# IsaacTroche1/MPC_ARPO_Project

Measured on AMD Instinct MI355X. Metric: MPC-QP solves/sec @ N=20, 6-state CW, batch=65536; ADMM iters to 1e-4, higher is better.
Workload: dtype f64

## Files before the change

mpc_arpo_project_amd/csrc/engine.hip:

```cpp
#include <hip/hip_runtime.h>

#include <algorithm>
#include <cmath>
#include <cstdio>
#include <cstdlib>
#include <cstring>
#include <string>
#include <vector>

#include "../../include/mpcqp.h"
#include "dev_plan.hpp"
#include "host_abi.hpp"
#include "symbolic.hpp"

using namespace mpcqp;

#pragma clang fp contract(off)

#define OSQP_INFTY 1e30
#define RHO_MIN 1e-06
#define RHO_MAX 1e06
#define RHO_EQ_OVER_RHO_INEQ 1e03
#define RHO_TOL 1e-04
#define MIN_SCALING 1e-04
// ... 1452 lines not shown
#pragma unroll
  for (int r = 0; r < RN; ++r) {
    const int j = lane + 64 * r;
    const double di = 1. / D[r];
    if (j < n) {
      v[P.S_DT + j] = di;
      qw[j] = (S.q[r] * cinv) * di;
    }
  }
  LDS_FENCE();
  unscale_p_r(v, P.S_P, P.nnzP, ra, ca, cinv, lane, Pw);
}

template <class Cx, int RN, int RM>
__device__ __forceinline__ void scale_bounds(const KParams& p, int inst, bool rebound, Inst<RN, RM>& S,
                                             const Slab& sb, const Cx& C, const double (&D)[RN],
                                             const double (&E)[RM]) {
  const DevPlan& P = p.pl;
  const int n = P.n, m = P.m, lane = C.lane;
  S.cinv = 1. / S.c;
  const double thr = OSQP_INFTY * MIN_SCALING;
  const double* Eold = p.Ecls + (size_t)inst * m;
  S.ct = 0;
#pragma unroll
  for (int r = 0; r < RM; ++r) {
    const int i = lane + 64 * (r + C.zo);
    const double ec = (rebound && i < m) ? Eold[i] : E[r];
    const double lc = S.l[r] * ec, uc = S.u[r] * ec;
    const uint32_t t = (lc < -thr && uc > thr) ? CT_FREE : ((uc - lc < RHO_TOL) ? CT_EQ : CT_INEQ);
    S.ct |= t << (2 * r);
    const double eci = 1. / ec;
    const double lb = rebound ? lc * eci : S.l[r], ub = rebound ? uc * eci : S.u[r];
    S.l[r] = lb * E[r];
    S.u[r] = ub * E[r];
    S.Einv[r] = 1. / E[r];
    if (i < m) sb.E[i] = E[r];
  }
#pragma unroll
  for (int r = 0; r < RN; ++r) {
    const int j = lane + 64 * (r + C.xo);
    S.Dinv[r] = 1. / D[r];
    if (j < n) sb.D[j] = D[r];
  }
}
template <int RN, int RM>
__device__ __forceinline__ void scale_finish(const KParams& p, int inst, bool rebound, Inst<RN, RM>& S,
                                             const Slab& sb, double* v, double* mvw, int lane,
                                             const double (&D)[RN], const double (&E)[RM]) {
  const DevPlan& P = p.pl;
  scale_bounds(p, inst, rebound, S, sb, One{lane, mvw}, D, E);
  LDS_FENCE();
  {
    const int cnt = P.nnzP + P.nnzA;
    constexpr int U = 8;
    for (int k0 = 0; k0 < cnt; k0 += 64 * U) {
      double x[U];
#pragma unroll
      for (int u = 0; u < U; ++u) {
        const int k = k0 + 64 * u + lane;
        x[u] = v[P.S_P + (k < cnt ? k : 0)];
      }
#pragma unroll
      for (int u = 0; u < U; ++u) {
        const int k = k0 + 64 * u + lane;
        if (k < cnt) mvw[P.MV + k] = x[u];
      }
    }
    if (lane == 0) mvw[P.MVZ] = 0.0;
  }
  LDS_FENCE();
  if (P.mv_slab) __builtin_amdgcn_fence(__ATOMIC_SEQ_CST, "workgroup");
}

#ifdef MPCQP_TIMING
#define TTAIL_PARAM , unsigned long long* tacc, unsigned long long t_tl
#define TTAIL_ARG(t) , tacc, t
#else
#define TTAIL_PARAM
#define TTAIL_ARG(t)
#endif
template <class Cx, int RN, int RM>
__device__ __forceinline__ void store_solution(const KParams& p, int inst, const Inst<RN, RM>& S,
                                               const Slab& sb, double* v, Cx& C, int status, int iter,
                                               int rho_updates TTAIL_PARAM) {
  const DevPlan& P = p.pl;
  const int n = P.n, m = P.m, lane = C.lane;
  const bool sol = has_solution(status);
  double obj = 0.0;
  if (sol) {
    double* xb = v + P.W;
    const double* mv = C.mv(v);
    LDS_FENCE();
#pragma unroll
    for (int r = 0; r < RN; ++r)
      if (lane + 64 * (r + C.xo) < n) xb[lane + 64 * (r + C.xo)] = S.x[r];
    C.sync(p, v);
    double part = 0.0;
    for (int k = C.tid(); k < P.nnzP; k += Cx::THREADS) {
      const int i = P.Pi[k], j = P.Pcol[k];
      const double pk = mv[P.MV + k];
      part += (i == j) ? .5 * pk * xb[i] * xb[i] : pk * xb[i] * xb[j];
    }
#pragma unroll
    for (int r = 0; r < RN; ++r)
      if (lane + 64 * (r + C.xo) < n) part += S.q[r] * S.x[r];
    obj = xch_sum(p, v, C, wave_sum(part)) * S.cinv;
  } else if (status == MPCQP_PRIMAL_INFEASIBLE || status == MPCQP_PRIMAL_INFEASIBLE_INACCURATE) {
    obj = OSQP_INFTY;
  } else if (status == MPCQP_DUAL_INFEASIBLE || status == MPCQP_DUAL_INFEASIBLE_INACCURATE) {
    obj = -OSQP_INFTY;
  }
  const double qnan = __builtin_nan("");
#pragma unroll
  for (int r = 0; r < RN; ++r) {
    const int j = lane + 64 * (r + C.xo);
    if (j < n) {
      if (p.x_out) p.x_out[(size_t)inst * n + j] = sol ? sb.D[j] * S.x[r] : qnan;
      p.xs[(size_t)inst * n + j] = sol ? S.x[r] : 0.0;
    }
  }
#pragma unroll
  for (int r = 0; r < RM; ++r) {
    const int i = lane + 64 * (r + C.zo);
    if (i < m) {
      const double Ei = sb.E[i];
      if (p.y_out) p.y_out[(size_t)inst * m + i] = sol ? (Ei * S.y[r]) * S.cinv : qnan;
      p.zs[(size_t)inst * m + i] = sol ? S.z[r] : 0.0;
      p.ys[(size_t)inst * m + i] = sol ? S.y[r] : 0.0;
      p.Ecls[(size_t)inst * m + i] = Ei;
    }
  }
  T_END(T_TAIL, t_tl);
#ifdef MPCQP_TIMING
  if (C.first() && p.timing)
    for (int k = 0; k < T_NSLOT; ++k) atomicAdd(p.timing + k, tacc[k]);
#endif
  if (C.first()) {
    p.rho_state[inst] = S.rho;
    p.has_state[inst] = 1;
    if (p.info.status) p.info.status[inst] = status;
    if (p.info.iter) p.info.iter[inst] = iter;
    if (p.info.rho_updates) p.info.rho_updates[inst] = rho_updates;
    if (p.info.obj_val) p.info.obj_val[inst] = obj;
    if (p.info.pri_res) p.info.pri_res[inst] = S.pri_res;
    if (p.info.dua_res) p.info.dua_res[inst] = S.dua_res;
    if (p.info.rho) p.info.rho[inst] = S.rho;
  }
}

#ifndef MPCQP_OPAQUE_LANE_RN
#define MPCQP_OPAQUE_LANE_RN 2
#endif
enum { KM_LDS = 0, KM_MATPF = 1, KM_MVG = 2, KM_MREG = 3 };
template <int RN, int RM, bool PAIRED, int KM, int RP>
__device__ __forceinline__ void solve_instance(const KParams& p, int inst, double* v, double* scr,
                                               int lane) {
  constexpr bool MATPF = KM == KM_MATPF, MVG = KM == KM_MVG, MREG = KM == KM_MREG;
  constexpr bool CARRY = RP == RP_CARRY;
  static_assert(!CARRY || KM == KM_LDS, "the carried record pipeline is the KM_LDS kernel's");
  const DevPlan& P = p.pl;
  const int n = P.n, m = P.m;
  const Slab sb = slab_of(P, scr);
  double* const mv = MVG ? sb.MV : v;
  One W{lane, mv};
  Inst<RN, RM> S;
  const int hs = p.has_state[inst];
  const Drift dr = drift_of(p, inst);
#ifdef MPCQP_TIMING
  unsigned long long tacc[T_NSLOT] = {};
#endif
  T_BEGIN(t_sc);
  {
    double D[RN], E[RM];
    scale_problem<RN, RM>(p, inst, dr, S, v, lane, D, E TACC_ARG);
    T_BEGIN(t_sf);
    scale_finish<RN, RM>(p, inst, dr.rebound, S, sb, v, mv, lane, D, E);
    if (lane == 0) {
      p.dsel[inst] = dr.sel;
      p.pend[inst] = 0;
    }
    T_END(T_SCFIN, t_sf);
  }
  T_END(T_SCALE, t_sc);
  S.rho = (hs != 0) ? p.rho_state[inst] : p.rho0;
  set_rho(S);
  T_BEGIN(t_f0);
  MatRegs M;
  assemble_and_factor<RN, RM>(p, sb, v, mv, lane, S);
  if constexpr (MREG) {
    LDS_FENCE();
    load_mats(P.fwdm, P.nfwd, (uint32_t)lane, v, M.m[0]);
    load_mats(P.bwdm, P.nbwd, (uint32_t)lane, v, M.m[1]);
  }
  T_END(T_FACTOR, t_f0);
  T_COUNT(T_NFACT);

  const bool warm = p.s.warm_start && hs != 0;
  if (warm && hs == 1) {
#pragma unroll
    for (int r = 0; r < RN; ++r) {
      const int j = lane + 64 * r;
      S.x[r] = j < n ? p.xs[(size_t)inst * n + j] : 0.0;
    }
#pragma unroll
    for (int r = 0; r < RM; ++r) {
      const int i = lane + 64 * r;
      S.z[r] = i < m ? p.zs[(size_t)inst * m + i] : 0.0;
      S.y[r] = i < m ? p.ys[(size_t)inst * m + i] : 0.0;
    }
  } else if (warm && hs == 2) {
#pragma unroll
    for (int r = 0; r < RN; ++r) {
      const int j = lane + 64 * r;
      S.x[r] = j < n ? S.Dinv[r] * p.xs[(size_t)inst * n + j] : 0.0;
    }
#pragma unroll
    for (int r = 0; r < RM; ++r) {
      const int i = lane + 64 * r;
      S.y[r] = i < m ? (S.Einv[r] * p.ys[(size_t)inst * m + i]) * S.c : 0.0;
    }
    double* xb = v + P.W;
    LDS_FENCE();
#pragma unroll
    for (int r = 0; r < RN; ++r)
      if (lane + 64 * r < n) xb[lane + 64 * r] = S.x[r];
    LDS_FENCE();
    double az[RM];
    ell_mv<RM, ELL_KA>(P.eA, mv, xb, az, W, W.zo, W.stage(P, v));
#pragma unroll
    for (int r = 0; r < RM; ++r) S.z[r] = lane + 64 * r < m ? az[r] : 0.0;
    LDS_FENCE();
  } else {
#pragma unroll
    for (int r = 0; r < RN; ++r) S.x[r] = 0.0;
#pragma unroll
    for (int r = 0; r < RM; ++r) S.z[r] = 0.0, S.y[r] = 0.0;
  }
  S.pri_res = S.dua_res = 0.0;

  int wsx[RN], wsz[RM];
#pragma unroll
  for (int r = 0; r < RN; ++r) wsx[r] = (int)P.wsx[lane + 64 * r];
#pragma unroll
  for (int r = 0; r < RM; ++r) wsz[r] = (int)P.wsz[lane + 64 * r];
  constexpr int coff = 64 * (RN + RM);
  const uint32_t wcp = P.wcopy[lane], bcp = P.bcopy[lane];
  constexpr bool MASK_REGS = RN < 4;
  constexpr int NMK = MASK_REGS ? RN + RM : 1;
  uint32_t wmk[NMK], bmk[NMK];
#pragma unroll
  for (int r = 0; r < NMK; ++r) {
    wmk[r] = 0u - ((wcp >> r) & 1u);
    bmk[r] = 0u - ((bcp >> r) & 1u);
    asm volatile("" : "+v"(wmk[r]), "+v"(bmk[r]));
  }
  auto slot_mask = [&](const uint32_t (&arr)[NMK], uint32_t bits, int r) -> uint32_t {
    if constexpr (MASK_REGS) return arr[r];
    return (uint32_t)((int32_t)(bits << (31 - r)) >> 31);
  };
  auto and_d = [](double x, uint32_t mk) {
    return __hiloint2double((int)((uint32_t)__double2hiint(x) & mk), (int)((uint32_t)__double2loint(x) & mk));
  };
  double sigma = p.s.sigma, alpha = p.s.alpha, alpha_c = 1.0 - p.s.alpha;
  asm volatile("" : "+v"(sigma), "+v"(alpha), "+v"(alpha_c));
  const int chk = p.s.check_termination;
  int ar_int = p.s.adaptive_rho_interval;
  if (p.s.adaptive_rho && ar_int == 0) ar_int = chk ? 4 * chk : 100;
  if (!p.s.adaptive_rho) ar_int = 0;
  int chk_left = chk, ar_left = ar_int;
  int status = MPCQP_UNSOLVED, iter = 0, rho_updates = 0;
  bool can_check = false;
  double dx[RN], dy[RM];
  Resid<RN, RM> R;
  Pipe<SolveOps<PAIRED>> sp;
  PipeC spc;
  const SolveOps<PAIRED> sops{v};
  const Rsrc rs_fwd = MREG    ? table_rsrc(P.fwdc, P.nfwd, SOLVEC_STEP_WORDS)
                      : CARRY ? carry_rsrc(P)
                              : table_rsrc(P.fwd, P.nfwd, SOLVE_STEP_WORDS);
  const Rsrc rs_bwd = MREG    ? table_rsrc(P.bwdc, P.nbwd, SOLVEC_STEP_WORDS)
                      : CARRY ? rs_fwd
                              : table_rsrc(P.bwd, P.nbwd, SOLVE_STEP_WORDS);
  int nfwd_s = P.nfwd, nbwd_s = P.nbwd;
  if constexpr (CARRY) asm volatile("" : "+s"(nfwd_s), "+s"(nbwd_s));
  constexpr bool DREG = RN == 2 && !MREG;
  double dvr[DREG ? RN + RM : 1];
  auto load_dinv = [&](int ln) {
    if constexpr (DREG) {
      LDS_FENCE();
#pragma unroll
      for (int r = 0; r < RN + RM; ++r) dvr[r] = v[P.DINV + ln + 64 * r];
    }
  };
  load_dinv(lane);
  int max_iter = p.s.max_iter;
  int chk_s = chk, ar_s = ar_int;
  asm volatile("" : "+s"(max_iter), "+s"(chk_s), "+s"(ar_s));
  if constexpr (CARRY) carry_restart(rs_fwd, P.nfwd, (uint32_t)lane, sp);
  for (iter = 1; iter <= max_iter; ++iter) {
    T_COUNT(T_ITERS);
    T_BEGIN(t_v0);
    if constexpr (MREG)
      prefetch_c(rs_fwd, P.nfwd, (uint32_t)lane, spc);
    else if constexpr (!CARRY)
      prefetch(rs_fwd, P.nfwd, (uint32_t)lane, sp);
    double xp[RN], zp[RM], bz[RM];
    uint32_t wbits = wcp, bbits = bcp;
    if constexpr (!MASK_REGS) asm volatile("" : "+v"(wbits), "+v"(bbits));
#pragma unroll
    for (int r = 0; r < RN; ++r) {
      xp[r] = S.x[r];
      const double b = fma(sigma, xp[r], -S.q[r]);
      v[wsx[r] + coff] = b;
      v[wsx[r]] = and_d(b, slot_mask(wmk, wbits, r));
    }
#pragma unroll
    for (int r = 0; r < RM; ++r) {
      zp[r] = S.z[r];
      bz[r] = fma(-rinv_of(S, r), S.y[r], zp[r]);
      v[wsz[r] + coff] = bz[r];
      v[wsz[r]] = and_d(bz[r], slot_mask(wmk, wbits, RN + r));
    }
    LDS_FENCE();
    T_END(T_VEC, t_v0);
    T_END(T_V0, t_v0);
    T_BEGIN(t_fw);
    if constexpr (MREG)
      run_body_r<PAIRED>(rs_fwd, P.nfwd, (uint32_t)lane, v, spc, M.m[0]);
    else if constexpr (MATPF)
      run_body_pf<PAIRED>(rs_fwd, P.nfwd, (uint32_t)lane, v, sp);
    else if constexpr (CARRY)
      run_body_carry<PAIRED>(rs_fwd, 0, nfwd_s, (uint32_t)lane, v, sp);
    else
      run_body(rs_fwd, P.nfwd, (uint32_t)lane, sops, sp);
    T_END(T_FWD, t_fw);
    T_BEGIN(t_v1);
    if constexpr (MREG)
      prefetch_c(rs_bwd, P.nbwd, (uint32_t)lane, spc);
    else if constexpr (!CARRY)
      prefetch(rs_bwd, P.nbwd, (uint32_t)lane, sp);
    {
      double wv[RN + RM], dv[RN + RM];
#pragma unroll
      for (int r = 0; r < RN + RM; ++r) {
        wv[r] = v[P.W + lane + 64 * r];
        if constexpr (DREG)
          dv[r] = dvr[r];
        else
          dv[r] = v[P.DINV + lane + 64 * r];
      }
#pragma unroll
      for (int r = 0; r < RN + RM; ++r) {
        const double c = wv[r] * dv[r];
        v[P.W + lane + 64 * r + coff] = c;
        v[P.W + lane + 64 * r] = and_d(c, slot_mask(bmk, bbits, r));
      }
    }
    LDS_FENCE();
    T_END(T_VEC, t_v1);
    T_END(T_V1, t_v1);
    T_BEGIN(t_bw);
    if constexpr (MREG)
      run_body_r<PAIRED>(rs_bwd, P.nbwd, (uint32_t)lane, v, spc, M.m[1]);
    else if constexpr (MATPF)
      run_body_pf<PAIRED>(rs_bwd, P.nbwd, (uint32_t)lane, v, sp);
    else if constexpr (CARRY)
      run_body_carry<PAIRED>(rs_fwd, nfwd_s, nbwd_s, (uint32_t)lane, v, sp);
    else
      run_body(rs_bwd, P.nbwd, (uint32_t)lane, sops, sp);
    T_END(T_BWD, t_bw);
    T_BEGIN(t_v2);
    double wx[RN], wz[RM];
#pragma unroll
    for (int r = 0; r < RN; ++r) wx[r] = v[wsx[r]];
#pragma unroll
    for (int r = 0; r < RM; ++r) wz[r] = v[wsz[r]];
    __builtin_amdgcn_sched_group_barrier(0x100, RN + RM, 0);
#pragma unroll
    for (int r = 0; r < RN; ++r) {
      const double xt = wx[r];
      S.x[r] = fma(alpha, xt, alpha_c * xp[r]);
      dx[r] = S.x[r] - xp[r];
    }
#pragma unroll
    for (int r = 0; r < RM; ++r) {
      const double nu = wz[r];
      const double ri = rinv_of(S, r);
      const double zt = fma(ri, nu, bz[r]);
      const double zr = fma(alpha, zt, alpha_c * zp[r]);
      S.z[r] = dmind(dmaxd(fma(ri, S.y[r], zr), S.l[r]), S.u[r]);
      dy[r] = rvec_of(S, r) * (zr - S.z[r]);
      S.y[r] = S.y[r] + dy[r];
    }
    LDS_FENCE();
    T_END(T_VEC, t_v2);
    T_END(T_V2, t_v2);
    T_BEGIN(t_ck);
    can_check = chk_s && --chk_left == 0;
    if (can_check) chk_left = chk_s;
    const bool adapt = ar_s && --ar_left == 0;
    if (adapt) ar_left = ar_s;
    int clane = lane;
    if constexpr (RN >= MPCQP_OPAQUE_LANE_RN) asm volatile("" : "+v"(clane));
    One C{clane, mv};
    if (can_check || adapt) {
      T_BEGIN(t_rs);
      compute_residuals(p, S, R, v, C TACC_ARG);
      T_END(T_RESID, t_rs);
      T_COUNT(T_NCHK);
    }
    if (can_check) {
      T_BEGIN(t_tm);
      status = check_termination(p, S, R, dy, dx, sb, v, C, false TACC_ARG);
      T_END(T_TERM, t_tm);
      if (status != 0) break;
      status = MPCQP_UNSOLVED;
    }
    T_BEGIN(t_ad);
    if (adapt) {
      const double rho_new = rho_estimate(p, S, R, v, C);
      if (rho_new > S.rho * p.s.adaptive_rho_tolerance ||
          rho_new < S.rho / p.s.adaptive_rho_tolerance) {
        S.rho = dmind(dmaxd(rho_new, RHO_MIN), RHO_MAX);
        set_rho(S);
        rho_updates++;
        LDS_FENCE();
        T_BEGIN(t_f1);
        assemble_and_factor<RN, RM>(p, sb, v, mv, clane, S);
        if constexpr (MREG) {
          LDS_FENCE();
          load_mats(P.fwdm, P.nfwd, (uint32_t)clane, v, M.m[0]);
          load_mats(P.bwdm, P.nbwd, (uint32_t)clane, v, M.m[1]);
        }
        load_dinv(clane);
#ifdef MPCQP_TIMING
        const unsigned long long dt_f1 = __builtin_amdgcn_s_memtime() - t_f1;
        tacc[T_FACTOR] += dt_f1;
        tacc[T_CHECK] -= dt_f1;
        tacc[T_ADAPT] -= dt_f1;
        tacc[T_RS2] -= dt_f1;
#endif
        T_COUNT(T_NFACT);
      }
    }
    T_END(T_ADAPT, t_ad);
    if constexpr (CARRY) {
      if (can_check || adapt) carry_restart(rs_fwd, P.nfwd, (uint32_t)lane, sp);
    }
    T_END(T_CHECK, t_ck);
#ifdef MPCQP_TIMING
    tacc[(can_check || adapt) ? T_RS2 : T_RS3] += __builtin_amdgcn_s_memtime() - t_ck;
#endif
  }
  T_BEGIN(t_tl);
  if (!can_check) {
    iter = iter - 1;
    compute_residuals(p, S, R, v, W TACC_ARG);
    status = check_termination(p, S, R, dy, dx, sb, v, W, false TACC_ARG);
    if (status == 0) status = MPCQP_UNSOLVED;
  }
  if (iter > p.s.max_iter) iter = p.s.max_iter;
  if (status == MPCQP_UNSOLVED) {
    const int st = check_termination(p, S, R, dy, dx, sb, v, W, true TACC_ARG);
    status = st ? st : MPCQP_MAX_ITER_REACHED;
  }

  store_solution(p, inst, S, sb, v, W, status, iter, rho_updates TTAIL_ARG(t_tl));
}

#ifndef MPCQP_WAVES_PER_EU
#define MPCQP_WAVES_PER_EU 1
#endif
template <int RN, int RM, bool PAIRED, int KM, int RP = RP_RESTART>
__global__ void __launch_bounds__(64, KM == KM_MVG ? 2 : MPCQP_WAVES_PER_EU) qp_batch_kernel(KParams p) {
  extern __shared__ __attribute__((aligned(16))) double lds[];
  const int lane = (int)threadIdx.x;
  if ((uint32_t)(uintptr_t)lds != 0u) __builtin_trap();
  double* v = lds;
  double* scr = p.scratch + (size_t)blockIdx.x * slab_doubles(p.pl);
  for (;;) {
    unsigned int inst = 0;
    if (lane == 0) inst = atomicAdd(p.counter, 1u);
    inst = (unsigned int)__shfl((int)inst, 0);
    inst = __builtin_amdgcn_readfirstlane(inst);
    if (inst >= (unsigned int)p.B) break;
    if (p.order) {
      inst = __builtin_amdgcn_readfirstlane((unsigned int)p.order[inst]);
      if (inst >= (unsigned int)p.B) continue;
    }
    if (p.skip && p.skip[inst]) continue;
    int ilane = lane;
    if constexpr (RN >= MPCQP_OPAQUE_LANE_RN) asm volatile("" : "+v"(ilane));
    solve_instance<RN, RM, PAIRED, KM, RP>(p, (int)inst, v, scr, ilane);
    LDS_FENCE();
  }
}

#ifndef MPCQP_PAIR_PIPE
#define MPCQP_PAIR_PIPE 4
#endif
constexpr int PAIR_PIPE = MPCQP_PAIR_PIPE;
#include "engine_pair.inc"

__global__ void bcast_rows_kernel(double* dst, const double* src, int B, int cnt) {
  const size_t t = (size_t)blockIdx.x * blockDim.x + threadIdx.x;
  if (t < (size_t)B * cnt) dst[t] = src[t % (size_t)cnt];
}

__global__ void drift_gather_kernel(double* dst, const double* W, const double* setup, int stride,
                                    const int32_t* dsel, int B, int cnt) {
  const size_t t = (size_t)blockIdx.x * blockDim.x + threadIdx.x;
  if (t >= (size_t)B * cnt) return;
  const size_t b = t / (size_t)cnt, k = t % (size_t)cnt;
  const int sel = dsel[b];
  dst[t] = sel == -2 ? setup[b * (size_t)stride + k] : W[(sel == 0 ? (size_t)B * cnt : 0) + t];
}

__global__ void update_P_kernel(double* setup, int setup_stride, double* W, const double* src,
                                int src_stride, const int32_t* dsel, int32_t* pend, int B, int cnt) {
  const size_t t = (size_t)blockIdx.x * blockDim.x + threadIdx.x;
  if (t >= (size_t)B * cnt) return;
  const size_t b = t / (size_t)cnt, k = t % (size_t)cnt;
  const int sel = dsel[b];
  const double val = src[b * (size_t)src_stride + k];
  if (sel == -2) {
    setup[b * (size_t)setup_stride + k] = val;
  } else {
    W[(sel == 0 ? (size_t)B * cnt : 0) + t] = val;
    if (k == 0) pend[b] = 1;
  }
}

#define HIPCHK(x)                                                                   \
  do {                                                                              \
    hipError_t e_ = (x);                                                            \
    if (e_ != hipSuccess) return set_error(MPCQP_E_HIP, std::string(#x) + ": " + hipGetErrorString(e_)); \
  } while (0)

typedef void (*kernel_fn)(KParams);

template <int RN, int RM>
kernel_fn pick(bool paired, int waves, bool matpf, bool mvg, bool mreg, bool carry) {
  if (waves == 3)
    return diag_env_int("MPCQP_W0DIAG", 0)
               ? (paired ? qp_pair_kernel<RN / 2, RM / 2, true, 3> : qp_pair_kernel<RN / 2, RM / 2, false, 3>)
               : (paired ? qp_pair_kernel<RN / 2, RM / 2, true, 2> : qp_pair_kernel<RN / 2, RM / 2, false, 2>);
  if (waves == 2) {
    if (matpf)
      return paired ? qp_pair_kernel<RN / 2, RM / 2, true, 1> : qp_pair_kernel<RN / 2, RM / 2, false, 1>;
    return paired ? qp_pair_kernel<RN / 2, RM / 2, true, 0> : qp_pair_kernel<RN / 2, RM / 2, false, 0>;
  }
  if (mvg || mreg) {
    if constexpr (RN == 2) {
      if (matpf || (mvg && mreg)) return nullptr;
      if (mreg)
        return paired ? qp_batch_kernel<RN, RM, true, KM_MREG> : qp_batch_kernel<RN, RM, false, KM_MREG>;
      return paired ? qp_batch_kernel<RN, RM, true, KM_MVG> : qp_batch_kernel<RN, RM, false, KM_MVG>;
    }
    return nullptr;
  }
  if (matpf)
    return paired ? qp_batch_kernel<RN, RM, true, KM_MATPF> : qp_batch_kernel<RN, RM, false, KM_MATPF>;
  if constexpr (RN == 2) {
    if (carry)
      return paired ? qp_batch_kernel<RN, RM, true, KM_LDS, RP_CARRY>
                    : qp_batch_kernel<RN, RM, false, KM_LDS, RP_CARRY>;
  }
  return paired ? qp_batch_kernel<RN, RM, true, KM_LDS> : qp_batch_kernel<RN, RM, false, KM_LDS>;
}

kernel_fn select_kernel(int n, int m, bool paired, int waves, bool matpf, bool mvg, bool mreg,
                        bool carry) {
  int rn = 0, rm = 0;
  if (!kernel_bucket(n, m, rn, rm)) return nullptr;
#ifdef MPCQP_DEV20
#ifdef MPCQP_DEV40
  if (rn == 4 && waves == 3 && !matpf && !mvg && !mreg)
    return paired ? qp_pair_kernel<2, 4, true, 2> : qp_pair_kernel<2, 4, false, 2>;
#endif
  if (rn != 2 || waves != 1 || matpf || mvg || mreg) return nullptr;
  if (carry)
    return paired ? qp_batch_kernel<2, 4, true, KM_LDS, RP_CARRY>
                  : qp_batch_kernel<2, 4, false, KM_LDS, RP_CARRY>;
  return paired ? qp_batch_kernel<2, 4, true, KM_LDS> : qp_batch_kernel<2, 4, false, KM_LDS>;
#else
  if (rn == 2) return pick<2, 4>(paired, waves, matpf, mvg, mreg, carry);
#ifndef MPCQP_ONLY_SMALL
  if (rn == 4) return pick<4, 8>(paired, waves, matpf, mvg, mreg, false);
#endif
  return nullptr;
#endif
}

constexpr int MREG_DEFAULT = 0;
bool use_mreg(const Plan& pl) {
  int rn = 0, rm = 0;
  const bool fits = pl.waves == 1 && !pl.mat_first && !pl.mv_global && pl.nfwd <= MREG_STEPS &&
                    pl.nbwd <= MREG_STEPS && kernel_bucket(pl.n, pl.m, rn, rm) && rn == 2;
  return fits && diag_env_int("MPCQP_MREG", MREG_DEFAULT) != 0;
}

bool record_carry(const Plan& pl, const DevImage& img) {
  int rn = 0, rm = 0;
  if (!img.carry || !kernel_bucket(pl.n, pl.m, rn, rm) || rn != 2) return false;
  const char* e = diag_env("MPCQP_RECORD_PIPE");
  return !(e && strcmp(e, "restart") == 0);
}

}

struct mpcqp_handle {
  Plan plan;
  mpcqp_settings set;
  int B = 0;
  hipStream_t stream = nullptr;
  std::vector<void*> owned;
  char* d_blob = nullptr;
  DevPlan dp{};
  double *Px = nullptr, *q = nullptr, *Ax = nullptr, *l = nullptr, *u = nullptr;
  double *PxB = nullptr, *qB = nullptr;
  bool batched = false;
  double *xs = nullptr, *zs = nullptr, *ys = nullptr, *rho = nullptr, *Ecls = nullptr;
  double *Pw = nullptr, *qw = nullptr;
  int32_t *dsel = nullptr, *pend = nullptr;
  bool a_inplace = false;
  int32_t* has_state = nullptr;
  double* scratch = nullptr;
  unsigned int* counter = nullptr;
  unsigned long long* timing = nullptr;
  bool has_data = false;
  const int32_t* skip = nullptr;
  const int32_t* order = nullptr;
  int grid = 0, lds_bytes = 0, waves_per_cu = 0, per_cu = 0;
  int kregs = 0, kscratch = 0;
  int block = 64;
  kernel_fn kern = nullptr;
};

template <typename T>
static bool dev_alloc(mpcqp_handle* h, T*& ptr, size_t bytes) {
  void* p = nullptr;
  if (hipMalloc(&p, bytes) != hipSuccess) return false;
  h->owned.push_back(ptr = (T*)p);
  return true;
}
template <typename T>
static hipError_t copy_rows(const mpcqp_handle* h, T* dst, const T* src, size_t count) {
  return hipMemcpyAsync(dst, src, sizeof(T) * count, hipMemcpyDeviceToDevice, h->stream);
}
template <typename... P, typename... A>
static hipError_t launch_1d(const mpcqp_handle* h, void (*kern)(P...), size_t elements, A... args) {
  if (elements == 0) return hipSuccess;
  hipLaunchKernelGGL(kern, dim3((unsigned)((elements + 255) / 256)), dim3(256), 0, h->stream, args...);
  return hipGetLastError();
}
static int guard(const mpcqp_handle* h, bool args = true, const char* what = nullptr) {
  if (!h || !args) return set_error(MPCQP_E_INVALID, h ? "null argument" : "null handle");
  if (what && !h->has_data) return set_error(MPCQP_E_NODATA, std::string(what) + " before set_data");
  return 0;
}
struct SetupRows {
  double *Px, *q;
  int Px_stride, q_stride;
};
static SetupRows setup_rows(const mpcqp_handle* h, bool batched) {
  return batched ? SetupRows{h->PxB, h->qB, h->plan.nnzP, h->plan.n} : SetupRows{h->Px, h->q, 0, 0};
}

extern "C" {

int mpcqp_create(const mpcqp_structure* st, const mpcqp_settings* s, int32_t batch, void* stream,
                 mpcqp_handle** out) {
  if (!st || !s || !out || batch <= 0) return set_error(MPCQP_E_INVALID, "invalid argument");
  *out = nullptr;
  if (st->m <= 0) return set_error(MPCQP_E_UNSUPPORTED, "problems without constraints (m == 0)");
  if (s->polish) return set_error(MPCQP_E_UNSUPPORTED, "polish is not implemented in this build");
  if (s->scaled_termination)
    return set_error(MPCQP_E_UNSUPPORTED, "scaled_termination is not implemented in this build");
  if (s->max_iter <= 0 || s->alpha <= 0 || s->alpha >= 2 || s->sigma <= 0 || s->rho <= 0 ||
      s->scaling < 0 || s->check_termination < 0 || s->eps_abs < 0 || s->eps_rel < 0)
    return set_error(MPCQP_E_INVALID, "invalid settings");
  mpcqp_handle* h = new mpcqp_handle();
  auto fail = [h](int code, std::string msg) { return mpcqp_destroy(h), set_error(code, msg); };
  h->set = *s;
  h->B = batch;
  h->stream = (hipStream_t)stream;
  if (!plan_for(st, h->plan)) return fail(MPCQP_E_UNSUPPORTED, h->plan.error);
  const Plan& pl = h->plan;
  h->block = 64 * pl.waves;

  const bool mreg = use_mreg(pl);
  DevImage img;
  std::string err;
  if (int rc = build_dev_image(pl, mreg, img, err)) return fail(rc, err);
  const bool carry = record_carry(pl, img);
  if (const char* e = diag_env("MPCQP_RECORD_PIPE"); e && strcmp(e, "carry") == 0 && !carry)
    return fail(MPCQP_E_UNSUPPORTED, "MPCQP_RECORD_PIPE=carry: this plan's record pipeline cannot be carried");
  h->kern = select_kernel(pl.n, pl.m, pl.paired, pl.waves == 2 ? (pl.split_steps ? 2 : 3) : 1,
                          pl.mat_first, pl.mv_global, mreg, carry);
  if (!h->kern) return fail(MPCQP_E_UNSUPPORTED, "problem dimensions exceed the instantiated kernels");
  if (!dev_alloc(h, h->d_blob, img.blob.size())) return fail(MPCQP_E_HIP, "hipMalloc(structure)");
  if (hipMemcpy(h->d_blob, img.blob.data(), img.blob.size(), hipMemcpyHostToDevice) != hipSuccess)
    return fail(MPCQP_E_HIP, "hipMemcpy(structure)");
  rebase(img, h->d_blob);
  h->dp = img.dp;

  int dev = 0, ncu = 0;
  if (hipGetDevice(&dev) != hipSuccess) return fail(MPCQP_E_HIP, "hipGetDevice");
  if (hipDeviceGetAttribute(&ncu, hipDeviceAttributeMultiprocessorCount, dev) != hipSuccess)
    return fail(MPCQP_E_HIP, "hipDeviceGetAttribute");
  const int inst_bytes = h->dp.inst_doubles * 8;
  const int lds_cap = 160 * 1024;
  const int lds_alloc = inst_bytes + std::max(0, diag_env_int("MPCQP_LDS_PAD", 0));
  if (lds_alloc > lds_cap) return fail(MPCQP_E_UNSUPPORTED, "instance image exceeds the LDS of a CU");
  if (hipFuncSetAttribute((const void*)h->kern, hipFuncAttributeMaxDynamicSharedMemorySize,
                          lds_cap) != hipSuccess)
    return fail(MPCQP_E_HIP, "hipFuncSetAttribute");
  hipFuncAttributes fa{};
  if (hipFuncGetAttributes(&fa, (const void*)h->kern) != hipSuccess)
    return fail(MPCQP_E_HIP, "hipFuncGetAttributes");
  h->kregs = fa.numRegs;
  h->kscratch = (int)fa.localSizeBytes;
  if (h->kregs > diag_env_int("MPCQP_REG_BUDGET", MPCQP_MAX_KERNEL_REGS) ||
      h->kscratch > MPCQP_MAX_KERNEL_SCRATCH)
    return fail(MPCQP_E_UNSUPPORTED,
                "solve kernel allocates " + std::to_string(h->kregs) + " registers / " +
                    std::to_string(h->kscratch) + " scratch bytes per lane: above the validated budget");
  int nb = 0;
  if (hipOccupancyMaxActiveBlocksPerMultiprocessor(&nb, (const void*)h->kern, h->block, lds_alloc) !=
          hipSuccess || nb <= 0)
    return fail(MPCQP_E_UNSUPPORTED, "kernel does not fit on a CU (LDS/VGPR)");
  h->per_cu = nb;
  h->waves_per_cu = nb * pl.waves;
  h->lds_bytes = lds_alloc;
  h->grid = std::min(batch, nb * ncu);

  const size_t Bz = (size_t)batch, D = sizeof(double), I = sizeof(int32_t);
  const size_t nP = (size_t)std::max(1, pl.nnzP), nA = (size_t)std::max(1, pl.nnzA);
  const bool ok = dev_alloc(h, h->Px, D * nP) && dev_alloc(h, h->q, D * pl.n) &&
                  dev_alloc(h, h->Ax, D * Bz * nA) && dev_alloc(h, h->l, D * Bz * pl.m) &&
                  dev_alloc(h, h->u, D * Bz * pl.m) && dev_alloc(h, h->xs, D * Bz * pl.n) &&
                  dev_alloc(h, h->zs, D * Bz * pl.m) && dev_alloc(h, h->ys, D * Bz * pl.m) &&
                  dev_alloc(h, h->Ecls, D * Bz * pl.m) && dev_alloc(h, h->Pw, 2 * D * Bz * nP) &&
                  dev_alloc(h, h->qw, 2 * D * Bz * pl.n) && dev_alloc(h, h->dsel, I * Bz) &&
                  dev_alloc(h, h->pend, I * Bz) && dev_alloc(h, h->rho, D * Bz) &&
                  dev_alloc(h, h->has_state, I * Bz) &&
                  dev_alloc(h, h->scratch, D * (size_t)h->grid * slab_doubles(pl.n, pl.m, pl.mv_slab)) &&
                  dev_alloc(h, h->counter, 64);
  if (!ok) return fail(MPCQP_E_HIP, "hipMalloc(batch buffers)");
  if (hipMemset(h->has_state, 0, I * Bz) != hipSuccess || hipMemsetD32(h->dsel, -2, Bz) != hipSuccess ||
      hipMemset(h->pend, 0, I * Bz) != hipSuccess)
    return fail(MPCQP_E_HIP, "hipMemset");
  *out = h;
  return 0;
}

int mpcqp_destroy(mpcqp_handle* h) {
  if (!h) return 0;
  for (void* p : h->owned) (void)hipFree(p);
  delete h;
  return 0;
}

static hipError_t bcast_rows(mpcqp_handle* h, double* dst, const double* src, int cnt) {
  return launch_1d(h, bcast_rows_kernel, (size_t)h->B * cnt, dst, src, h->B, cnt);
}

static int batched_rows(mpcqp_handle* h) {
  const size_t B = (size_t)h->B;
  if ((!h->PxB && !dev_alloc(h, h->PxB, sizeof(double) * B * std::max(1, h->plan.nnzP))) ||
      (!h->qB && !dev_alloc(h, h->qB, sizeof(double) * B * h->plan.n)))
    return set_error(MPCQP_E_HIP, "hipMalloc(per-instance cost rows)");
  return 0;
}
static int promote(mpcqp_handle* h) {
  if (h->batched) return 0;
  if (int rc = batched_rows(h)) return rc;
  HIPCHK(bcast_rows(h, h->PxB, h->Px, h->plan.nnzP));
  HIPCHK(bcast_rows(h, h->qB, h->q, h->plan.n));
  h->batched = true;
  return 0;
}

static int set_data(mpcqp_handle* h, bool batched, const double* Px, const double* q,
                    const double* Ax, const double* l, const double* u) {
  if (int rc = guard(h, Px && q && Ax && l && u)) return rc;
  if (int rc = batched ? batched_rows(h) : 0) return rc;
  const Plan& pl = h->plan;
  const size_t B = (size_t)h->B, rows = batched ? B : 1;
  const SetupRows to = setup_rows(h, batched);
  HIPCHK(copy_rows(h, to.Px, Px, rows * pl.nnzP));
  HIPCHK(copy_rows(h, to.q, q, rows * pl.n));
  HIPCHK(copy_rows(h, h->Ax, Ax, B * pl.nnzA));
  HIPCHK(copy_rows(h, h->l, l, B * pl.m));
  HIPCHK(copy_rows(h, h->u, u, B * pl.m));
  HIPCHK(hipMemsetAsync(h->has_state, 0, sizeof(int32_t) * B, h->stream));
  HIPCHK(hipMemsetD32Async(h->dsel, -2, B, h->stream));
  HIPCHK(hipMemsetAsync(h->pend, 0, sizeof(int32_t) * B, h->stream));
  h->has_data = true;
  h->batched = batched;
  return 0;
}

int mpcqp_set_data(mpcqp_handle* h, const double* Px, const double* q, const double* Ax,
                   const double* l, const double* u) {
  return set_data(h, false, Px, q, Ax, l, u);
}

int mpcqp_set_data_batched(mpcqp_handle* h, const double* Px, const double* q, const double* Ax,
                           const double* l, const double* u) {
  return set_data(h, true, Px, q, Ax, l, u);
}

int mpcqp_update_bounds(mpcqp_handle* h, const double* l, const double* u) {
  if (int rc = guard(h, l && u, "update")) return rc;
  const size_t Bm = (size_t)h->B * h->plan.m;
  HIPCHK(copy_rows(h, h->l, l, Bm));
  HIPCHK(copy_rows(h, h->u, u, Bm));
  return 0;
}

int mpcqp_update_A(mpcqp_handle* h, const double* Ax) {
  if (int rc = guard(h, Ax, "update")) return rc;
  HIPCHK(copy_rows(h, h->Ax, Ax, (size_t)h->B * h->plan.nnzA));
  HIPCHK(hipMemsetD32Async(h->pend, 1, (size_t)h->B, h->stream));
  return 0;
}

int mpcqp_update_lin_cost(mpcqp_handle* h, const double* q) {
  if (int rc = guard(h, q, "update")) return rc;
  const int n = h->plan.n;
  HIPCHK(copy_rows(h, h->q, q, n));
  if (h->batched) HIPCHK(bcast_rows(h, h->qB, h->q, n));
  HIPCHK(bcast_rows(h, h->qw, h->q, n));
  HIPCHK(bcast_rows(h, h->qw + (size_t)h->B * n, h->q, n));
  return 0;
}

int mpcqp_update_lin_cost_batched(mpcqp_handle* h, const double* q) {
  if (int rc = guard(h, q, "update")) return rc;
  if (int rc = promote(h)) return rc;
  const size_t Bn = (size_t)h->B * h->plan.n;
  HIPCHK(copy_rows(h, h->qB, q, Bn));
  HIPCHK(copy_rows(h, h->qw, q, Bn));
  HIPCHK(copy_rows(h, h->qw + Bn, q, Bn));
  return 0;
}

static int update_P(mpcqp_handle* h, const double* Px, int src_stride) {
  const int cnt = h->plan.nnzP;
  const SetupRows s = setup_rows(h, h->batched);
  HIPCHK(launch_1d(h, update_P_kernel, (size_t)h->B * cnt, s.Px, s.Px_stride, h->Pw, Px, src_stride,
                   h->dsel, h->pend, h->B, cnt));
  return 0;
}

int mpcqp_update_P(mpcqp_handle* h, const double* Px) {
  if (int rc = guard(h, Px, "update")) return rc;
  return update_P(h, Px, 0);
}

int mpcqp_update_P_batched(mpcqp_handle* h, const double* Px) {
  if (int rc = guard(h, Px, "update")) return rc;
  if (int rc = promote(h)) return rc;
  return update_P(h, Px, h->plan.nnzP);
}

int mpcqp_warm_start(mpcqp_handle* h, const double* x, const double* y) {
  if (int rc = guard(h, x && y, "warm start")) return rc;
  const size_t B = (size_t)h->B;
  HIPCHK(copy_rows(h, h->xs, x, B * h->plan.n));
  HIPCHK(copy_rows(h, h->ys, y, B * h->plan.m));
  HIPCHK(hipMemsetD32Async(h->has_state, 2, B, h->stream));
  HIPCHK(hipStreamSynchronize(h->stream));
  return 0;
}

int mpcqp_solve(mpcqp_handle* h, double* x, double* y, const mpcqp_info* info) {
  if (int rc = guard(h, true, "solve")) return rc;
  const SetupRows s = setup_rows(h, h->batched);
  KParams p{};
  p.pl = h->dp;
  p.s = h->set;
  p.B = h->B;
  p.Px = s.Px, p.q = s.q, p.Px_stride = s.Px_stride, p.q_stride = s.q_stride;
  p.Ax = h->Ax, p.l = h->l, p.u = h->u;
  p.xs = h->xs, p.zs = h->zs, p.ys = h->ys, p.rho_state = h->rho, p.Ecls = h->Ecls;
  p.Pw = h->Pw, p.qw = h->qw;
  p.dsel = h->dsel, p.pend = h->pend, p.a_inplace = h->a_inplace ? 1 : 0;
  p.has_state = h->has_state;
  p.x_out = x, p.y_out = y;
  if (info) p.info = *info;
  p.scratch = h->scratch;
  p.counter = h->counter;
  p.timing = h->timing;
  p.rho0 = std::min(std::max(h->set.rho, RHO_MIN), RHO_MAX);
  p.skip = h->skip;
  p.order = h->order;
  HIPCHK(hipMemsetAsync(h->counter, 0, 64, h->stream));
  hipLaunchKernelGGL(h->kern, dim3(h->grid), dim3(h->block), h->lds_bytes, h->stream, p);
  HIPCHK(hipGetLastError());
  return 0;
}

#ifdef MPCQP_TIMING
int mpcqp_debug_timing(mpcqp_handle* h, unsigned long long* dev_buf) {
  if (int rc = guard(h)) return rc;
  h->timing = dev_buf;
  return 0;
}
#endif

#ifdef MPCQP_PAIR_CHECKS
int mpcqp_debug_pair_inject(int on) {
  return hipMemcpyToSymbol(HIP_SYMBOL(g_pair_inject), &on, sizeof(int)) == hipSuccess ? 0 : MPCQP_E_HIP;
}
#endif

int mpcqp_data_buffers(mpcqp_handle* h, double** Ax, double** l, double** u) {
  if (int rc = guard(h)) return rc;
  if (Ax) h->a_inplace = true;
  if (Ax) *Ax = h->Ax;
  if (l) *l = h->l;
  if (u) *u = h->u;
  return 0;
}

int mpcqp_copy_data(mpcqp_handle* h, double* Ax, double* l, double* u) {
  if (int rc = guard(h)) return rc;
  const size_t B = (size_t)h->B;
  if (Ax) HIPCHK(copy_rows(h, Ax, h->Ax, B * h->plan.nnzA));
  if (l) HIPCHK(copy_rows(h, l, h->l, B * h->plan.m));
  if (u) HIPCHK(copy_rows(h, u, h->u, B * h->plan.m));
  return 0;
}

int mpcqp_set_skip(mpcqp_handle* h, const int32_t* skip) {
  if (int rc = guard(h)) return rc;
  h->skip = skip;
  return 0;
}

int mpcqp_set_order(mpcqp_handle* h, const int32_t* order) {
  if (int rc = guard(h)) return rc;
  h->order = order;
  return 0;
}

int mpcqp_get_state(const mpcqp_handle* h, double* xs, double* zs, double* ys, double* rho,
// ... 95 lines not shown
```

Baseline: 879,200.

## Rotate ADMM loop in carry kernel so RHS formation follows the update

For the carried-record (CARRY) kernel, the ADMM iteration loop is rotated: the right-hand side is formed once before the loop and then at the end of each iteration right after the x/z/y update, with fast and check paths split. This drops the xp/zp temporaries and the per-iteration mask-opacity asm, and restarts the carry pipeline only on check iterations. The goal is to cut per-iteration register pressure and scheduling overhead in the hot loop. It also adds a kernel that resets per-instance rho on set_data and changes how the last-checked flag is tracked. The rotated path assumes check_termination and adaptive rho are both enabled, since the counters are decremented without the zero guards.

```diff
diff --git a/mpc_arpo_project_amd/csrc/engine.hip b/mpc_arpo_project_amd/csrc/engine.hip
--- a/mpc_arpo_project_amd/csrc/engine.hip
+++ b/mpc_arpo_project_amd/csrc/engine.hip
@@ -1628,6 +1628,9 @@
 #define MPCQP_OPAQUE_LANE_RN 2
 #endif
 enum { KM_LDS = 0, KM_MATPF = 1, KM_MVG = 2, KM_MREG = 3 };
+#ifndef MPCQP_ROTATE_LOOP
+#define MPCQP_ROTATE_LOOP 1
+#endif
 template <int RN, int RM, bool PAIRED, int KM, int RP>
 __device__ __forceinline__ void solve_instance(const KParams& p, int inst, double* v, double* scr,
                                                int lane) {
@@ -1745,7 +1748,6 @@
   if (!p.s.adaptive_rho) ar_int = 0;
   int chk_left = chk, ar_left = ar_int;
   int status = MPCQP_UNSOLVED, iter = 0, rho_updates = 0;
-  bool can_check = false;
   double dx[RN], dy[RM];
   Resid<RN, RM> R;
   Pipe<SolveOps<PAIRED>> sp;
@@ -1773,163 +1775,310 @@
   int chk_s = chk, ar_s = ar_int;
   asm volatile("" : "+s"(max_iter), "+s"(chk_s), "+s"(ar_s));
   if constexpr (CARRY) carry_restart(rs_fwd, P.nfwd, (uint32_t)lane, sp);
-  for (iter = 1; iter <= max_iter; ++iter) {
-    T_COUNT(T_ITERS);
-    T_BEGIN(t_v0);
-    if constexpr (MREG)
-      prefetch_c(rs_fwd, P.nfwd, (uint32_t)lane, spc);
-    else if constexpr (!CARRY)
-      prefetch(rs_fwd, P.nfwd, (uint32_t)lane, sp);
-    double xp[RN], zp[RM], bz[RM];
-    uint32_t wbits = wcp, bbits = bcp;
-    if constexpr (!MASK_REGS) asm volatile("" : "+v"(wbits), "+v"(bbits));
-#pragma unroll
-    for (int r = 0; r < RN; ++r) {
-      xp[r] = S.x[r];
-      const double b = fma(sigma, xp[r], -S.q[r]);
-      v[wsx[r] + coff] = b;
-      v[wsx[r]] = and_d(b, slot_mask(wmk, wbits, r));
-    }
-#pragma unroll
-    for (int r = 0; r < RM; ++r) {
-      zp[r] = S.z[r];
-      bz[r] = fma(-rinv_of(S, r), S.y[r], zp[r]);
-      v[wsz[r] + coff] = bz[r];
-      v[wsz[r]] = and_d(bz[r], slot_mask(wmk, wbits, RN + r));
-    }
-    LDS_FENCE();
-    T_END(T_VEC, t_v0);
-    T_END(T_V0, t_v0);
-    T_BEGIN(t_fw);
-    if constexpr (MREG)
-      run_body_r<PAIRED>(rs_fwd, P.nfwd, (uint32_t)lane, v, spc, M.m[0]);
-    else if constexpr (MATPF)
-      run_body_pf<PAIRED>(rs_fwd, P.nfwd, (uint32_t)lane, v, sp);
-    else if constexpr (CARRY)
+  constexpr bool ROTATE = CARRY && MPCQP_ROTATE_LOOP;
+  bool last_checked;
+  if constexpr (ROTATE) {
+    double bz[RM];
+    auto form_rhs = [&]() {
+      T_BEGIN(t_v0);
+#pragma unroll
+      for (int r = 0; r < RN; ++r) {
+        const double b = fma(sigma, S.x[r], -S.q[r]);
+        v[wsx[r] + coff] = b;
+        v[wsx[r]] = and_d(b, slot_mask(wmk, wcp, r));
+      }
+#pragma unroll
+      for (int r = 0; r < RM; ++r) {
+        bz[r] = fma(-rinv_of(S, r), S.y[r], S.z[r]);
+        v[wsz[r] + coff] = bz[r];
+        v[wsz[r]] = and_d(bz[r], slot_mask(wmk, wcp, RN + r));
+      }
+      LDS_FENCE();
+      T_END(T_VEC, t_v0);
+      T_END(T_V0, t_v0);
+    };
+    auto update_xzy = [&]() {
+      T_BEGIN(t_v2);
+      double wx[RN], wz[RM];
+#pragma unroll
+      for (int r = 0; r < RN; ++r) wx[r] = v[wsx[r]];
+#pragma unroll
+      for (int r = 0; r < RM; ++r) wz[r] = v[wsz[r]];
+      __builtin_amdgcn_sched_group_barrier(0x100, RN + RM, 0);
+#pragma unroll
+      for (int r = 0; r < RN; ++r) {
+        const double xt = wx[r], xp = S.x[r];
+        S.x[r] = fma(alpha, xt, alpha_c * xp);
+        dx[r] = S.x[r] - xp;
+      }
+#pragma unroll
+      for (int r = 0; r < RM; ++r) {
+        const double nu = wz[r];
+        const double ri = rinv_of(S, r);
+        const double zt = fma(ri, nu, bz[r]);
+        const double zr = fma(alpha, zt, alpha_c * S.z[r]);
+        S.z[r] = dmind(dmaxd(fma(ri, S.y[r], zr), S.l[r]), S.u[r]);
+        dy[r] = rvec_of(S, r) * (zr - S.z[r]);
+        S.y[r] = S.y[r] + dy[r];
+      }
+      LDS_FENCE();
+      T_END(T_VEC, t_v2);
+      T_END(T_V2, t_v2);
+    };
+    form_rhs();
+    for (iter = 1; iter <= max_iter; ++iter) {
+      T_COUNT(T_ITERS);
+      T_BEGIN(t_fw);
       run_body_carry<PAIRED>(rs_fwd, 0, nfwd_s, (uint32_t)lane, v, sp);
-    else
-      run_body(rs_fwd, P.nfwd, (uint32_t)lane, sops, sp);
-    T_END(T_FWD, t_fw);
-    T_BEGIN(t_v1);
-    if constexpr (MREG)
-      prefetch_c(rs_bwd, P.nbwd, (uint32_t)lane, spc);
-    else if constexpr (!CARRY)
-      prefetch(rs_bwd, P.nbwd, (uint32_t)lane, sp);
-    {
-      double wv[RN + RM], dv[RN + RM];
-#pragma unroll
-      for (int r = 0; r < RN + RM; ++r) {
-        wv[r] = v[P.W + lane + 64 * r];
-        if constexpr (DREG)
-          dv[r] = dvr[r];
-        else
-          dv[r] = v[P.DINV + lane + 64 * r];
+      T_END(T_FWD, t_fw);
+      T_BEGIN(t_v1);
+      {
+        double wv[RN + RM], dv[RN + RM];
+#pragma unroll
+        for (int r = 0; r < RN + RM; ++r) {
+          wv[r] = v[P.W + lane + 64 * r];
+          if constexpr (DREG)
+            dv[r] = dvr[r];
+          else
+            dv[r] = v[P.DINV + lane + 64 * r];
+        }
+#pragma unroll
+        for (int r = 0; r < RN + RM; ++r) {
+          const double c = wv[r] * dv[r];
+          v[P.W + lane + 64 * r + coff] = c;
+          v[P.W + lane + 64 * r] = and_d(c, slot_mask(bmk, bcp, r));
+        }
       }
-#pragma unroll
-      for (int r = 0; r < RN + RM; ++r) {
-        const double c = wv[r] * dv[r];
-        v[P.W + lane + 64 * r + coff] = c;
-        v[P.W + lane + 64 * r] = and_d(c, slot_mask(bmk, bbits, r));
+      LDS_FENCE();
+      T_END(T_VEC, t_v1);
+      T_END(T_V1, t_v1);
+      T_BEGIN(t_bw);
+      run_body_carry<PAIRED>(rs_fwd, nfwd_s, nbwd_s, (uint32_t)lane, v, sp);
+      T_END(T_BWD, t_bw);
+      T_BEGIN(t_c0);
+      const bool can_check = --chk_left == 0;
+      const bool adapt = --ar_left == 0;
+      if (!(can_check || adapt)) {
+        T_END(T_CHECK, t_c0);
+        T_END(T_RS3, t_c0);
+        update_xzy();
+        form_rhs();
+      } else {
+        if (can_check) chk_left = chk_s;
+        if (adapt) ar_left = ar_s;
+        T_END(T_CHECK, t_c0);
+        T_END(T_RS2, t_c0);
+        update_xzy();
+        __builtin_amdgcn_sched_barrier(0);
+        T_BEGIN(t_ck);
+        int clane = lane;
+        if constexpr (RN >= MPCQP_OPAQUE_LANE_RN) asm volatile("" : "+v"(clane));
+        One C{clane, mv};
+        {
+          T_BEGIN(t_rs);
+          compute_residuals(p, S, R, v, C TACC_ARG);
+          T_END(T_RESID, t_rs);
+          T_COUNT(T_NCHK);
+        }
+        if (can_check) {
+          T_BEGIN(t_tm);
+          status = check_termination(p, S, R, dy, dx, sb, v, C, false TACC_ARG);
+          T_END(T_TERM, t_tm);
+          if (status != 0) break;
+          status = MPCQP_UNSOLVED;
+        }
+        T_BEGIN(t_ad);
+        if (adapt) {
+          const double rho_new = rho_estimate(p, S, R, v, C);
+          if (rho_new > S.rho * p.s.adaptive_rho_tolerance ||
+              rho_new < S.rho / p.s.adaptive_rho_tolerance) {
+            S.rho = dmind(dmaxd(rho_new, RHO_MIN), RHO_MAX);
+            set_rho(S);
+            rho_updates++;
+            LDS_FENCE();
+            T_BEGIN(t_f1);
+            assemble_and_factor<RN, RM>(p, sb, v, mv, clane, S);
+            load_dinv(clane);
+#ifdef MPCQP_TIMING
+            const unsigned long long dt_f1 = __builtin_amdgcn_s_memtime() - t_f1;
+            tacc[T_FACTOR] += dt_f1;
+            tacc[T_CHECK] -= dt_f1;
+            tacc[T_ADAPT] -= dt_f1;
+            tacc[T_RS2] -= dt_f1;
+#endif
+            T_COUNT(T_NFACT);
+          }
+        }
+        T_END(T_ADAPT, t_ad);
+        carry_restart(rs_fwd, P.nfwd, (uint32_t)lane, sp);
+        T_END(T_CHECK, t_ck);
+        T_END(T_RS2, t_ck);
+        form_rhs();
       }
-    }
-    LDS_FENCE();
-    T_END(T_VEC, t_v1);
-    T_END(T_V1, t_v1);
-    T_BEGIN(t_bw);
-    if constexpr (MREG)
-      run_body_r<PAIRED>(rs_bwd, P.nbwd, (uint32_t)lane, v, spc, M.m[1]);
-    else if constexpr (MATPF)
-      run_body_pf<PAIRED>(rs_bwd, P.nbwd, (uint32_t)lane, v, sp);
-    else if constexpr (CARRY)
-      run_body_carry<PAIRED>(rs_fwd, nfwd_s, nbwd_s, (uint32_t)lane, v, sp);
-    else
-      run_body(rs_bwd, P.nbwd, (uint32_t)lane, sops, sp);
-    T_END(T_BWD, t_bw);
-    T_BEGIN(t_v2);
-    double wx[RN], wz[RM];
-#pragma unroll
-    for (int r = 0; r < RN; ++r) wx[r] = v[wsx[r]];
-#pragma unroll
-    for (int r = 0; r < RM; ++r) wz[r] = v[wsz[r]];
-    __builtin_amdgcn_sched_group_barrier(0x100, RN + RM, 0);
-#pragma unroll
-    for (int r = 0; r < RN; ++r) {
-      const double xt = wx[r];
-      S.x[r] = fma(alpha, xt, alpha_c * xp[r]);
-      dx[r] = S.x[r] - xp[r];
-    }
-#pragma unroll
-    for (int r = 0; r < RM; ++r) {
-      const double nu = wz[r];
-      const double ri = rinv_of(S, r);
-      const double zt = fma(ri, nu, bz[r]);
-      const double zr = fma(alpha, zt, alpha_c * zp[r]);
-      S.z[r] = dmind(dmaxd(fma(ri, S.y[r], zr), S.l[r]), S.u[r]);
-      dy[r] = rvec_of(S, r) * (zr - S.z[r]);
-      S.y[r] = S.y[r] + dy[r];
-    }
-    LDS_FENCE();
-    T_END(T_VEC, t_v2);
-    T_END(T_V2, t_v2);
-    T_BEGIN(t_ck);
-    can_check = chk_s && --chk_left == 0;
-    if (can_check) chk_left = chk_s;
-    const bool adapt = ar_s && --ar_left == 0;
-    if (adapt) ar_left = ar_s;
-    int clane = lane;
-    if constexpr (RN >= MPCQP_OPAQUE_LANE_RN) asm volatile("" : "+v"(clane));
-    One C{clane, mv};
-    if (can_check || adapt) {
-      T_BEGIN(t_rs);
-      compute_residuals(p, S, R, v, C TACC_ARG);
-      T_END(T_RESID, t_rs);
-      T_COUNT(T_NCHK);
-    }
-    if (can_check) {
-      T_BEGIN(t_tm);
-      status = check_termination(p, S, R, dy, dx, sb, v, C, false TACC_ARG);
-      T_END(T_TERM, t_tm);
-      if (status != 0) break;
-      status = MPCQP_UNSOLVED;
-    }
-    T_BEGIN(t_ad);
-    if (adapt) {
-      const double rho_new = rho_estimate(p, S, R, v, C);
-      if (rho_new > S.rho * p.s.adaptive_rho_tolerance ||
-          rho_new < S.rho / p.s.adaptive_rho_tolerance) {
-        S.rho = dmind(dmaxd(rho_new, RHO_MIN), RHO_MAX);
-        set_rho(S);
-        rho_updates++;
-        LDS_FENCE();
-        T_BEGIN(t_f1);
-        assemble_and_factor<RN, RM>(p, sb, v, mv, clane, S);
-        if constexpr (MREG) {
+      LDS_FENCE();
+    }
+    last_checked = status != MPCQP_UNSOLVED || (iter > 1 && chk_left == chk_s);
+  } else {
+    bool can_check = false;
+    for (iter = 1; iter <= max_iter; ++iter) {
+      T_COUNT(T_ITERS);
+      T_BEGIN(t_v0);
+      if constexpr (MREG)
+        prefetch_c(rs_fwd, P.nfwd, (uint32_t)lane, spc);
+      else if constexpr (!CARRY)
+        prefetch(rs_fwd, P.nfwd, (uint32_t)lane, sp);
+      double xp[RN], zp[RM], bz[RM];
+      uint32_t wbits = wcp, bbits = bcp;
+      if constexpr (!MASK_REGS) asm volatile("" : "+v"(wbits), "+v"(bbits));
+#pragma unroll
+      for (int r = 0; r < RN; ++r) {
+        xp[r] = S.x[r];
+        const double b = fma(sigma, xp[r], -S.q[r]);
+        v[wsx[r] + coff] = b;
+        v[wsx[r]] = and_d(b, slot_mask(wmk, wbits, r));
+      }
+#pragma unroll
+      for (int r = 0; r < RM; ++r) {
+        zp[r] = S.z[r];
+        bz[r] = fma(-rinv_of(S, r), S.y[r], zp[r]);
+        v[wsz[r] + coff] = bz[r];
+        v[wsz[r]] = and_d(bz[r], slot_mask(wmk, wbits, RN + r));
+      }
+      LDS_FENCE();
+      T_END(T_VEC, t_v0);
+      T_END(T_V0, t_v0);
+      T_BEGIN(t_fw);
+      if constexpr (MREG)
+        run_body_r<PAIRED>(rs_fwd, P.nfwd, (uint32_t)lane, v, spc, M.m[0]);
+      else if constexpr (MATPF)
+        run_body_pf<PAIRED>(rs_fwd, P.nfwd, (uint32_t)lane, v, sp);
+      else if constexpr (CARRY)
+        run_body_carry<PAIRED>(rs_fwd, 0, nfwd_s, (uint32_t)lane, v, sp);
+      else
+        run_body(rs_fwd, P.nfwd, (uint32_t)lane, sops, sp);
+      T_END(T_FWD, t_fw);
+      T_BEGIN(t_v1);
+      if constexpr (MREG)
+        prefetch_c(rs_bwd, P.nbwd, (uint32_t)lane, spc);
+      else if constexpr (!CARRY)
+        prefetch(rs_bwd, P.nbwd, (uint32_t)lane, sp);
+      {
+        double wv[RN + RM], dv[RN + RM];
+#pragma unroll
+        for (int r = 0; r < RN + RM; ++r) {
+          wv[r] = v[P.W + lane + 64 * r];
+          if constexpr (DREG)
+            dv[r] = dvr[r];
+          else
+            dv[r] = v[P.DINV + lane + 64 * r];
+        }
+#pragma unroll
+        for (int r = 0; r < RN + RM; ++r) {
+          const double c = wv[r] * dv[r];
+          v[P.W + lane + 64 * r + coff] = c;
+          v[P.W + lane + 64 * r] = and_d(c, slot_mask(bmk, bbits, r));
+        }
+      }
+      LDS_FENCE();
+      T_END(T_VEC, t_v1);
+      T_END(T_V1, t_v1);
+      T_BEGIN(t_bw);
+      if constexpr (MREG)
+        run_body_r<PAIRED>(rs_bwd, P.nbwd, (uint32_t)lane, v, spc, M.m[1]);
+      else if constexpr (MATPF)
+        run_body_pf<PAIRED>(rs_bwd, P.nbwd, (uint32_t)lane, v, sp);
+      else if constexpr (CARRY)
+        run_body_carry<PAIRED>(rs_fwd, nfwd_s, nbwd_s, (uint32_t)lane, v, sp);
+      else
+        run_body(rs_bwd, P.nbwd, (uint32_t)lane, sops, sp);
+      T_END(T_BWD, t_bw);
+      T_BEGIN(t_v2);
+      double wx[RN], wz[RM];
+#pragma unroll
+      for (int r = 0; r < RN; ++r) wx[r] = v[wsx[r]];
+#pragma unroll
+      for (int r = 0; r < RM; ++r) wz[r] = v[wsz[r]];
+      __builtin_amdgcn_sched_group_barrier(0x100, RN + RM, 0);
+#pragma unroll
+      for (int r = 0; r < RN; ++r) {
+        const double xt = wx[r];
+        S.x[r] = fma(alpha, xt, alpha_c * xp[r]);
+        dx[r] = S.x[r] - xp[r];
+      }
+#pragma unroll
+      for (int r = 0; r < RM; ++r) {
+        const double nu = wz[r];
+        const double ri = rinv_of(S, r);
+        const double zt = fma(ri, nu, bz[r]);
+        const double zr = fma(alpha, zt, alpha_c * zp[r]);
+        S.z[r] = dmind(dmaxd(fma(ri, S.y[r], zr), S.l[r]), S.u[r]);
+        dy[r] = rvec_of(S, r) * (zr - S.z[r]);
+        S.y[r] = S.y[r] + dy[r];
+      }
+      LDS_FENCE();
+      T_END(T_VEC, t_v2);
+      T_END(T_V2, t_v2);
+      T_BEGIN(t_ck);
+      can_check = chk_s && --chk_left == 0;
+      if (can_check) chk_left = chk_s;
+      const bool adapt = ar_s && --ar_left == 0;
+      if (adapt) ar_left = ar_s;
+      int clane = lane;
+      if constexpr (RN >= MPCQP_OPAQUE_LANE_RN) asm volatile("" : "+v"(clane));
+      One C{clane, mv};
+      if (can_check || adapt) {
+        T_BEGIN(t_rs);
+        compute_residuals(p, S, R, v, C TACC_ARG);
+        T_END(T_RESID, t_rs);
+        T_COUNT(T_NCHK);
+      }
+      if (can_check) {
+        T_BEGIN(t_tm);
+        status = check_termination(p, S, R, dy, dx, sb, v, C, false TACC_ARG);
+        T_END(T_TERM, t_tm);
+        if (status != 0) break;
+        status = MPCQP_UNSOLVED;
+      }
+      T_BEGIN(t_ad);
+      if (adapt) {
+        const double rho_new = rho_estimate(p, S, R, v, C);
+        if (rho_new > S.rho * p.s.adaptive_rho_tolerance ||
+            rho_new < S.rho / p.s.adaptive_rho_tolerance) {
+          S.rho = dmind(dmaxd(rho_new, RHO_MIN), RHO_MAX);
+          set_rho(S);
+          rho_updates++;
           LDS_FENCE();
-          load_mats(P.fwdm, P.nfwd, (uint32_t)clane, v, M.m[0]);
-          load_mats(P.bwdm, P.nbwd, (uint32_t)clane, v, M.m[1]);
+          T_BEGIN(t_f1);
+          assemble_and_factor<RN, RM>(p, sb, v, mv, clane, S);
+          if constexpr (MREG) {
+            LDS_FENCE();
+            load_mats(P.fwdm, P.nfwd, (uint32_t)clane, v, M.m[0]);
+            load_mats(P.bwdm, P.nbwd, (uint32_t)clane, v, M.m[1]);
+          }
+          load_dinv(clane);
+#ifdef MPCQP_TIMING
+          const unsigned long long dt_f1 = __builtin_amdgcn_s_memtime() - t_f1;
+          tacc[T_FACTOR] += dt_f1;
+          tacc[T_CHECK] -= dt_f1;
+          tacc[T_ADAPT] -= dt_f1;
+          tacc[T_RS2] -= dt_f1;
+#endif
+          T_COUNT(T_NFACT);
         }
-        load_dinv(clane);
+      }
+      T_END(T_ADAPT, t_ad);
+      if constexpr (CARRY) {
+        if (can_check || adapt) carry_restart(rs_fwd, P.nfwd, (uint32_t)lane, sp);
+      }
+      T_END(T_CHECK, t_ck);
 #ifdef MPCQP_TIMING
-        const unsigned long long dt_f1 = __builtin_amdgcn_s_memtime() - t_f1;
-        tacc[T_FACTOR] += dt_f1;
-        tacc[T_CHECK] -= dt_f1;
-        tacc[T_ADAPT] -= dt_f1;
-        tacc[T_RS2] -= dt_f1;
+      tacc[(can_check || adapt) ? T_RS2 : T_RS3] += __builtin_amdgcn_s_memtime() - t_ck;
 #endif
-        T_COUNT(T_NFACT);
-      }
-    }
-    T_END(T_ADAPT, t_ad);
-    if constexpr (CARRY) {
-      if (can_check || adapt) carry_restart(rs_fwd, P.nfwd, (uint32_t)lane, sp);
-    }
-    T_END(T_CHECK, t_ck);
-#ifdef MPCQP_TIMING
-    tacc[(can_check || adapt) ? T_RS2 : T_RS3] += __builtin_amdgcn_s_memtime() - t_ck;
-#endif
+    }
+    last_checked = can_check;
   }
   T_BEGIN(t_tl);
-  if (!can_check) {
+  if (!last_checked) {
     iter = iter - 1;
     compute_residuals(p, S, R, v, W TACC_ARG);
     status = check_termination(p, S, R, dy, dx, sb, v, W, false TACC_ARG);
@@ -1981,6 +2130,11 @@
 __global__ void bcast_rows_kernel(double* dst, const double* src, int B, int cnt) {
   const size_t t = (size_t)blockIdx.x * blockDim.x + threadIdx.x;
   if (t < (size_t)B * cnt) dst[t] = src[t % (size_t)cnt];
+}
+
+__global__ void fill_kernel(double* dst, double x, size_t B) {
+  const size_t t = (size_t)blockIdx.x * blockDim.x + threadIdx.x;
+  if (t < B) dst[t] = x;
 }
 
 __global__ void drift_gather_kernel(double* dst, const double* W, const double* setup, int stride,
@@ -2271,6 +2425,7 @@
   HIPCHK(copy_rows(h, h->l, l, B * pl.m));
   HIPCHK(copy_rows(h, h->u, u, B * pl.m));
   HIPCHK(hipMemsetAsync(h->has_state, 0, sizeof(int32_t) * B, h->stream));
+  HIPCHK(launch_1d(h, fill_kernel, B, h->rho, std::min(std::max(h->set.rho, RHO_MIN), RHO_MAX), B));
   HIPCHK(hipMemsetD32Async(h->dsel, -2, B, h->stream));
   HIPCHK(hipMemsetAsync(h->pend, 0, sizeof(int32_t) * B, h->stream));
   h->has_data = true;
```

Result: faster. 907,200, median of 6 (+3.2%).
